# codgodtao/TMDiff

Measured on AMD Instinct MI355X. Metric: UNet denoise-steps/sec (8-ch 64x64, batch 32), higher is better.
Workload: dtype f32; 1 GPU; BASELINE configs[1]: batch-32 8-ch 64x64 tiles, DDPM p_sample steps of the T=1000 cosine schedule, channel_multiplier [32,64,128,256], full UNet forward (both branches) + fused DDPM update per step; batch_per_gpu=32, parallelism=batch-parallel x1, weights=key-hashed random init, text_embedding=fixed synthetic 768-d

## Files before the change

include/tmdiff_hip.h:

```cpp
#ifndef TMDIFF_HIP_H
#define TMDIFF_HIP_H

#include <stddef.h>
#include <stdint.h>

#ifdef __cplusplus
extern "C" {
#endif

#define TMDIFF_ABI_VERSION 6

#define TMDIFF_OK 0
#define TMDIFF_E_INVALID (-1)
#define TMDIFF_E_UNSUPPORTED (-2)
#define TMDIFF_E_LAUNCH (-3)

typedef void* tmdiff_stream_t;

int tmdiff_version(void);
const char* tmdiff_last_error_string(void);

typedef struct tmdiff_conv3d_desc {
  int32_t B, N, H, W;
  int32_t Cin, Cout;
// ... 81 lines not shown
int tmdiff_conv3d_wino_fwd(const tmdiff_conv3d_desc* d, void* workspace, tmdiff_stream_t stream);
int tmdiff_conv3d_wino_fwd_stage(const tmdiff_conv3d_desc* d, void* workspace, int32_t stage, tmdiff_stream_t stream);
int tmdiff_conv3d_wino_fwd_xp(const tmdiff_conv3d_desc* d, void* workspace, int32_t stage, float* xp_out, tmdiff_stream_t stream);
int tmdiff_conv3d_wino_fwd_planes(const tmdiff_conv3d_desc* d, void* workspace, int32_t stage, float* xp_out, int32_t planes,
                                  tmdiff_stream_t stream);

int tmdiff_conv3d_wf_supported(const tmdiff_conv3d_desc* d);
int64_t tmdiff_conv3d_wf_blocks(const tmdiff_conv3d_desc* d);
size_t tmdiff_conv3d_wf_splitk_workspace_bytes(const tmdiff_conv3d_desc* d);
size_t tmdiff_conv3d_wf_workspace_bytes(const tmdiff_conv3d_desc* d);
int32_t tmdiff_conv3d_wf_plan(int32_t B, int32_t Cin, int32_t Cout, int32_t N, int32_t H, int32_t W, int32_t groups, int32_t llm,
                              int64_t* tiles);
int tmdiff_conv3d_wf_fwd(const tmdiff_conv3d_desc* d, void* workspace, tmdiff_stream_t stream);

int tmdiff_conv3d_w2_supported(const tmdiff_conv3d_desc* d);
size_t tmdiff_conv3d_w2_workspace_bytes(const tmdiff_conv3d_desc* d);
size_t tmdiff_conv3d_w2_packed_bytes(int32_t Cout, int32_t Cin);
int tmdiff_conv3d_w2_pack_weights(const float* w, float* packed, int32_t Cout, int32_t Cin, tmdiff_stream_t stream);
int tmdiff_conv3d_w2_fwd(const tmdiff_conv3d_desc* d, void* workspace, int32_t stages, tmdiff_stream_t stream);
int tmdiff_conv3d_wfll_supported(const tmdiff_conv3d_desc* d);
size_t tmdiff_conv3d_wfll_packed_bytes(int32_t Cout, int32_t Cin);
int tmdiff_conv3d_wfll_pack_weights(const float* w, float* packed, int32_t Cout, int32_t Cin, float ll_scale,
                                    tmdiff_stream_t stream);
size_t tmdiff_conv3d_wfll_splitk_workspace_bytes(const tmdiff_conv3d_desc* d);
int tmdiff_conv3d_wfll_fwd(const tmdiff_conv3d_desc* d, float ll_scale, tmdiff_stream_t stream);

size_t tmdiff_conv3d_packed_bf16_bytes(int32_t Cout, int32_t Cin, int32_t ksize, int32_t groups);
int tmdiff_conv3d_pack_weights_bf16(const float* w, void* packed, int32_t Cout, int32_t Cin, int32_t ksize,
                                    int32_t groups, tmdiff_stream_t stream);
int tmdiff_conv3d_pack_weights_bf16_dgrad(const float* w, void* packed, int32_t Cout, int32_t Cin, int32_t ksize,
// ... 298 lines not shown
```

tmdiff_amd/Hyper_unet_general.py:

```python
import math

import torch
import torch.nn as nn

from . import ops, routing

PROMPTS = ("QB", "WV3", "GF2", "WV2", "WV4")

def synthetic_text_embeddings(seed=1234):
    out = {}
    for k, name in enumerate(PROMPTS):
        g = torch.Generator(device="cpu").manual_seed(seed + k)
        out[name] = torch.randn(1, 768, generator=g)
    return out


class Swish(nn.Module):

    def forward(self, x):
        raise RuntimeError("Swish is fused into the HIP kernels; it is never called as a module")



_MASK_FN = None
# ... 402 lines not shown
            y, y2 = self._conv(P, name + ".conv21", [t1], use_bias=False, residual=res, emit=emit, **self._own(pro21), **rckw)
            return (y, y2, None, plan.s2d) if want_ll else (y, y2)
        if side is not None:
            t1p = self._conv(P, name + ".conv20", [side], keep_y=False, emit=pro21)
        elif pre is not None:
            t1p = self._conv(P, name + ".conv20", [pre], keep_y=False, emit=pro21, x_bf16_shape=shape if pre.dtype == torch.int16 else None)
        else:
            t1p = self._conv(P, name + ".conv20", segs, keep_y=False, emit=pro21, **self._own(pro20))
        if plan.emit_ll:
            y2, yll = self._conv(P, name + ".conv21", [t1p], use_bias=False, residual=res, keep_y=False, emit=dict(emit, ll=True), **rckw)
            return None, y2, yll, plan.s2d
        y, y2 = self._conv(P, name + ".conv21", [t1p], use_bias=False, residual=res, emit=emit,
                           x_bf16_shape=shape if name + ".conv21" in P["bf16"] else None, **rckw)
        return (y, y2, None, plan.s2d) if want_ll else (y, y2)

    def _conv0(self, P, name, x, pre):
        if pre is None:
            return self._conv(P, name + ".Conv_0", [x], in_act=True, w2=False)
        return self._conv(P, name + ".Conv_0", [pre], x_bf16_shape=tuple(x.shape[2:]) if pre.dtype == torch.int16 else None, w2=False)

    def _down(self, P, S, name, x, flag, want_high, pre=None, emit=None, fuse=False, xq=None, s2d=False):
        shape = x.shape if x is not None else (*xq.shape[:3], 2 * xq.shape[3], 2 * xq.shape[4])
        plan = self._down_plan(P, name, shape, not want_high, pre is not None and pre.dtype == torch.float32, s2d, fuse)
        pro = self._spec(P, S, shift=None if flag else name + ".Dense_0", scale=name + ".dense1")
        if plan.conv0 == "dwt":
            hll, *bands = self._conv(P, name + ".Conv_0", [pre], keep_y=False, emit=dict(pro, dwt=True))
        elif plan.conv0 is None:
            hh = self._conv0(P, name, x, pre)
        rc2 = {}
        if not ops.config.conv2_after_ll:
            xll = ops.haar_dwt2d(self._conv(P, name + ".Conv_2", [x]), want_high=False, ll_scale=0.5)[0]
        else:
            if xq is None:
                xq = ops.haar_dwt2d(x, want_high=False, ll_scale=0.5)[0]
            if plan.fold:
                c2 = self.get_submodule(name + ".Conv_2")
                xll, rc2 = None, {"res_conv": (xq, c2.weight.detach(), xq.shape[1]), "bias": c2.bias.detach()}
            else:
                xll = self._conv(P, name + ".Conv_2", [xq])
        p16 = False
        if plan.conv0 in ("ll", "wfll"):
            c0, wfll = self.get_submodule(name + ".Conv_0"), plan.conv0 == "wfll"
            hll = (ops.conv3d_wf_ll if wfll else ops.conv3d_ll)(pre, P["w_wfll" if wfll else "w_ll"][name + ".Conv_0"], c0.out_channels, 0.5,
# ... 233 lines not shown
```

tmdiff_amd/_lib.py:

```python
import ctypes as C
import os

_HERE = os.path.dirname(os.path.abspath(__file__))
LIB_PATH = os.environ.get("TMDIFF_HIP_LIB") or os.path.join(_HERE, "libtmdiff_hip.so")

c_float_p = C.POINTER(C.c_float)
vp = C.c_void_p


class Conv3dDesc(C.Structure):
    _fields_ = [
        ("B", C.c_int32), ("N", C.c_int32), ("H", C.c_int32), ("W", C.c_int32),
        ("Cin", C.c_int32), ("Cout", C.c_int32),
        ("groups", C.c_int32), ("ksize", C.c_int32), ("nseg", C.c_int32),
        ("seg_c", C.c_int32 * 3),
        ("seg_x", vp * 3),
        ("w_packed", vp), ("bias", vp), ("bias_scale", C.c_float),
        ("in_shift", vp), ("in_scale", vp), ("in_shift_stride", C.c_int32), ("in_scale_stride", C.c_int32),
        ("in_mask", vp), ("in_act", C.c_int32),
        ("residual", vp), ("out_scale", C.c_float),
        ("y", vp),
        ("y2", vp), ("y2_shift", vp), ("y2_scale", vp), ("y2_shift_stride", C.c_int32), ("y2_scale_stride", C.c_int32),
        ("y2_act", C.c_int32), ("y2_bf16", C.c_int32), ("x_bf16", C.c_int32),
        ("splitk_ws", vp), ("splitk_ws_bytes", C.c_int64),
# ... 16 lines not shown
    "tmdiff_conv3d_fwd_staged": (C.c_int, [C.POINTER(Conv3dDesc), vp, vp]),
    "tmdiff_conv3d_wino_supported": (C.c_int, [C.POINTER(Conv3dDesc)]),
    "tmdiff_conv3d_wino_blocks": (C.c_int64, [C.POINTER(Conv3dDesc)]),
    "tmdiff_conv3d_wino_workspace_bytes": (C.c_size_t, [C.POINTER(Conv3dDesc)]),
    "tmdiff_conv3d_wino_planes": (C.c_int32, [C.c_int32]),
    "tmdiff_conv3d_wino_packed_bytes": (C.c_size_t, [C.c_int32, C.c_int32, C.c_int32, C.c_int32]),
    "tmdiff_conv3d_wino_pack_weights": (C.c_int, [vp, vp, C.c_int32, C.c_int32, C.c_int32, C.c_int32, C.c_int32, vp]),
    "tmdiff_conv3d_wino_pack_weights_multi_chunk": (C.c_int32, []),
    "tmdiff_conv3d_wino_pack_weights_multi": (C.c_int, [vp, vp, vp, C.c_int32, vp]),
    "tmdiff_conv3d_wf_supported": (C.c_int, [C.POINTER(Conv3dDesc)]),
    "tmdiff_conv3d_wf_blocks": (C.c_int64, [C.POINTER(Conv3dDesc)]),
    "tmdiff_conv3d_wf_workspace_bytes": (C.c_size_t, [C.POINTER(Conv3dDesc)]),
    "tmdiff_conv3d_wf_splitk_workspace_bytes": (C.c_size_t, [C.POINTER(Conv3dDesc)]),
    "tmdiff_conv3d_wf_fwd": (C.c_int, [C.POINTER(Conv3dDesc), vp, vp]),
    "tmdiff_conv3d_w2_supported": (C.c_int, [C.POINTER(Conv3dDesc)]),
    "tmdiff_conv3d_w2_workspace_bytes": (C.c_size_t, [C.POINTER(Conv3dDesc)]),
    "tmdiff_conv3d_w2_packed_bytes": (C.c_size_t, [C.c_int32, C.c_int32]),
    "tmdiff_conv3d_w2_pack_weights": (C.c_int, [vp, vp, C.c_int32, C.c_int32, vp]),
    "tmdiff_conv3d_w2_fwd": (C.c_int, [C.POINTER(Conv3dDesc), vp, C.c_int32, vp]),
    "tmdiff_conv3d_wino_fwd": (C.c_int, [C.POINTER(Conv3dDesc), vp, vp]),
    "tmdiff_conv3d_wino_fwd_planes": (C.c_int, [C.POINTER(Conv3dDesc), vp, C.c_int32, vp, C.c_int32, vp]),
    "tmdiff_conv3d_wino_fwd_xp": (C.c_int, [C.POINTER(Conv3dDesc), vp, C.c_int32, vp, vp]),
    "tmdiff_conv3d_wino_fwd_stage": (C.c_int, [C.POINTER(Conv3dDesc), vp, C.c_int32, vp]),
    "tmdiff_conv3d_prologue_fwd": (C.c_int, [C.POINTER(Conv3dDesc), vp, vp]),
    "tmdiff_conv3d_ll_supported": (C.c_int, [C.POINTER(Conv3dDesc)]),
    "tmdiff_conv3d_ll_splitk_workspace_bytes": (C.c_size_t, [C.POINTER(Conv3dDesc)]),
    "tmdiff_conv3d_ll_packed_bytes": (C.c_size_t, [C.c_int32, C.c_int32]),
    "tmdiff_conv3d_ll_pack_weights": (C.c_int, [vp, vp, C.c_int32, C.c_int32, C.c_float, vp]),
    "tmdiff_conv3d_ll_fwd": (C.c_int, [C.POINTER(Conv3dDesc), C.c_float, vp]),
    "tmdiff_conv3d_packed_bf16_bytes": (C.c_size_t, [C.c_int32, C.c_int32, C.c_int32, C.c_int32]),
# ... 189 lines not shown
```

tmdiff_amd/csrc/conv3d_w2.hip:

```cpp
#include "bufaddr.h"
#include "common.h"

namespace {

using namespace tmdiff;

constexpr int W2_XP = 384;
constexpr int W2_NP = 256;
constexpr int W2_KC = 16;
constexpr int W2_CO = 64;

struct W2Plan {
  int T, Q, TW, Hp, IP, OP;
  int G, ptiles;
  size_t xh_floats, mh_floats;
};

bool w2_shape_ok(const tmdiff_conv3d_desc* d) {
  if (!d || d->ksize != 3 || d->groups != 1 || d->x_bf16 || d->y2_bf16 || d->nseg != 1) return false;
  if (d->B <= 0 || (d->N != 4 && d->N != 8) || d->W < 2 || d->W > 16 || d->W % 2 || d->H < 4 || d->H > 32) return false;
  if (d->Cin < 128 || d->Cin % 32 || d->Cout < 256 || d->Cout % W2_CO || d->seg_c[0] != d->Cin) return false;
  if (d->in_mask || d->drop_p > 0.f || d->rc_x || d->rc_cin || d->y_ll || d->y_hi[0] || d->y2_s2d || d->xp_out) return false;
  return true;
}

W2Plan w2_plan(const tmdiff_conv3d_desc* d) {
  W2Plan p;
  p.T = d->N / 4; p.Q = d->B * p.T; p.TW = d->W / 2; p.Hp = d->H + 2;
  p.IP = p.Hp * p.TW; p.OP = d->H * p.TW;
  p.G = W2_NP / p.OP < W2_XP / p.IP ? W2_NP / p.OP : W2_XP / p.IP;
  if (p.G > p.Q) p.G = p.Q;
  p.ptiles = (p.Q + p.G - 1) / p.G;
  p.xh_floats = (size_t)24 * d->Cin * p.Q * p.IP;
  p.mh_floats = (size_t)24 * d->Cout * p.Q * p.OP;
  return p;
}

bool w2_fits(const tmdiff_conv3d_desc* d, const W2Plan& p) {
  const size_t xk = p.xh_floats / 24 * 4, mk = p.mh_floats / 24 * 4, uk = (size_t)3 * d->Cin * d->Cout * 4;
  return xk < (1ull << 31) && mk < (1ull << 31) && uk < (1ull << 31) && p.Q <= 65535 &&
         (long)p.ptiles * (d->Cout / W2_CO) * 24 < 0x7fffffffL;
}

__global__ void __launch_bounds__(256) w2_pack_kernel(const float* __restrict__ w, float* __restrict__ u, int Cout, int Cin) {
#pragma clang fp contract(off)
  const long idx = (long)blockIdx.x * 256 + threadIdx.x;
  if (idx >= (long)3 * Cin * Cout) return;
  const int e = idx & 3;
  long r = idx >> 2;
  const int co = r % Cout; r /= Cout;
  const int cq = r % (Cin / 4);
  const int dh = r / (Cin / 4);
  const int ci = cq * 4 + e;
  const float* src = w + ((long)co * Cin + ci) * 27 + dh * 3;
  float t[6][3];
// ... 211 lines not shown
}

struct W2OutArgs {
  const float* mh;
  const float* bias;
  float bias_scale;
  const float* residual;
  float out_scale;
  float* y;
  float* y2;
  const float* y2_shift;
  const float* y2_scale;
  int y2_shift_stride, y2_scale_stride, y2_act;
  int Cout, N, H, W, T, TW, OP;
  long QOP;
};

template <bool Y, bool RES, bool Y2>
__global__ void __launch_bounds__(256) w2_output_kernel(const W2OutArgs a) {
#pragma clang fp contract(off)
  __shared__ float tile[4 * 32 * 17];
  const int tid = threadIdx.x;
  const int cc = blockIdx.x, h = blockIdx.y, q = blockIdx.z;
  const int b = q / a.T, t = q % a.T;
  {
    const int co_l = tid & 31, tw = tid >> 5;
    if (tw < a.TW) {
      const float* src = a.mh + ((long)q * a.OP + h * a.TW + tw) * a.Cout + cc * 32 + co_l;
      const long kstride = a.QOP * a.Cout;
      float r[6][2];
// ... 39 lines not shown
    if constexpr (Y2) {
      const float sh2 = a.y2_shift ? a.y2_shift[(long)b * a.y2_shift_stride + co] : 0.f;
      const float sc2 = a.y2_scale ? a.y2_scale[(long)b * a.y2_scale_stride + co] : 1.f;
      float u[2];
#pragma unroll
      for (int e = 0; e < 2; ++e) {
        const float x = v[e] + sh2;
        const float xa = silu_f(x);
        u[e] = (a.y2_act ? xa : x) * sc2;
      }
      buf::store2(r2, o, make_float2(u[0], u[1]));
    }
  }
}

}

extern "C" int tmdiff_conv3d_w2_supported(const tmdiff_conv3d_desc* d) {
  return w2_shape_ok(d) && w2_fits(d, w2_plan(d)) ? 1 : 0;
}

extern "C" size_t tmdiff_conv3d_w2_workspace_bytes(const tmdiff_conv3d_desc* d) {
  if (!w2_shape_ok(d)) return 0;
  const W2Plan p = w2_plan(d);
  return (p.xh_floats + p.mh_floats) * sizeof(float);
}

extern "C" size_t tmdiff_conv3d_w2_packed_bytes(int32_t Cout, int32_t Cin) {
  if (Cout <= 0 || Cin <= 0 || Cin % 4) return 0;
  return (size_t)72 * Cout * Cin * sizeof(float);
}

extern "C" int tmdiff_conv3d_w2_pack_weights(const float* w, float* packed, int32_t Cout, int32_t Cin, tmdiff_stream_t stream) {
  using namespace tmdiff;
  TMDIFF_REQUIRE(w && packed, "conv3d_w2_pack_weights: NULL pointer");
  TMDIFF_REQUIRE(Cout > 0 && Cin > 0 && Cin % 4 == 0 && (size_t)72 * Cout * Cin < (1ull << 31),
                 "conv3d_w2_pack_weights: Cout=%d Cin=%d (Cin %% 4 == 0)", Cout, Cin);
  const long n = (long)3 * Cin * Cout;
  w2_pack_kernel<<<(unsigned)((n + 255) / 256), 256, 0, as_stream(stream)>>>(w, packed, Cout, Cin);
  return check_launch("conv3d_w2_pack_weights");
}

extern "C" int tmdiff_conv3d_w2_fwd(const tmdiff_conv3d_desc* d, void* workspace, int32_t stages, tmdiff_stream_t stream) {
  using namespace tmdiff;
  TMDIFF_REQUIRE(d && workspace, "conv3d_w2_fwd: NULL pointer");
  if (!w2_shape_ok(d))
    return fail(TMDIFF_E_UNSUPPORTED, "conv3d_w2_fwd: fp32 3x3x3, groups 1, one input tensor, 4 or 8 bands, even W <= 16, 4 <= H <= 32, "
                                      "Cin >= 128 (%% 32), Cout >= 256 (%% 64), plain y / y2 / residual epilogue");
  const W2Plan p = w2_plan(d);
  if (!w2_fits(d, p)) return fail(TMDIFF_E_UNSUPPORTED, "conv3d_w2_fwd: tensor too large for 32-bit offsets");
  TMDIFF_REQUIRE(d->seg_x[0] && d->w_packed && (d->y || d->y2), "conv3d_w2_fwd: input, weights and an output");
  TMDIFF_REQUIRE(aligned16(d->seg_x[0]) && aligned16(workspace) && aligned16(d->w_packed) && aligned16(d->y) && aligned16(d->y2) &&
                     aligned16(d->residual),
                 "conv3d_w2_fwd: 16-byte aligned tensors / workspace");
  hipStream_t st = as_stream(stream);
  float* xh = static_cast<float*>(workspace);
  float* mh = xh + p.xh_floats;
  if (stages == 0) stages = 7;

  if (stages & 1) {
    W2InArgs a;
    a.x = d->seg_x[0]; a.xh = xh;
    a.in_shift = d->in_shift; a.in_scale = d->in_scale;
    a.shift_stride = bank_stride(d->in_shift_stride, d->Cin);
    a.scale_stride = bank_stride(d->in_scale_stride, d->Cin);
    a.in_act = d->in_act;
    a.Cin = d->Cin; a.N = d->N; a.H = d->H; a.W = d->W; a.T = p.T; a.TW = p.TW; a.IP = p.IP;
    a.QIP = (long)p.Q * p.IP;
    w2_input_kernel<<<dim3((unsigned)(d->Cin / 32), (unsigned)p.Hp, (unsigned)p.Q), 256, 0, st>>>(a);
// ... 5 lines not shown
    a.Cin = d->Cin; a.Cout = d->Cout; a.Q = p.Q; a.TW = p.TW; a.IP = p.IP; a.OP = p.OP; a.G = p.G; a.ptiles = p.ptiles;
    a.cotiles = d->Cout / W2_CO;
    if (const int rc = set_grid(a, (long)p.ptiles * a.cotiles * 24, "conv3d_w2_fwd")) return rc;
    w2_gemm_kernel<<<a.total_blocks, 256, 0, st>>>(a);
    if (const int rc = check_launch("conv3d_w2_fwd")) return rc;
  }
  if (stages & 4) {
    W2OutArgs a;
    a.mh = mh;
    a.bias = d->bias; a.bias_scale = d->bias_scale; a.residual = d->residual; a.out_scale = d->out_scale;
    a.y = d->y; a.y2 = d->y2; a.y2_shift = d->y2_shift; a.y2_scale = d->y2_scale; a.y2_act = d->y2_act;
    a.y2_shift_stride = bank_stride(d->y2_shift_stride, d->Cout);
    a.y2_scale_stride = bank_stride(d->y2_scale_stride, d->Cout);
    a.Cout = d->Cout; a.N = d->N; a.H = d->H; a.W = d->W; a.T = p.T; a.TW = p.TW; a.OP = p.OP;
    a.QOP = (long)p.Q * p.OP;
    const dim3 grid((unsigned)(d->Cout / 32), (unsigned)d->H, (unsigned)p.Q);
#define TMDIFF_W2_OUT(Y, R, Y2) w2_output_kernel<Y, R, Y2><<<grid, 256, 0, st>>>(a)
    if (d->y) {
      if (d->residual) { if (d->y2) TMDIFF_W2_OUT(true, true, true); else TMDIFF_W2_OUT(true, true, false); }
      else             { if (d->y2) TMDIFF_W2_OUT(true, false, true); else TMDIFF_W2_OUT(true, false, false); }
    } else {
      if (d->residual) TMDIFF_W2_OUT(false, true, true); else TMDIFF_W2_OUT(false, false, true);
    }
#undef TMDIFF_W2_OUT
    if (const int rc = check_launch("conv3d_w2_fwd(output pass)")) return rc;
  }
  return TMDIFF_OK;
}
```

tmdiff_amd/ops.py:

```python
import collections
import ctypes as C
import math
import os

import numpy as np
import torch

from . import _lib, routing
from ._lib import Conv3dDesc, check, lib



class KernelConfig:

    _FLAG = lambda default: (lambda v: (v != "0") if default else (v == "1"))
    _FIELDS = {
        "winograd": ("TMDIFF_WINOGRAD", _FLAG(True), True), "wf": ("TMDIFF_WF", _FLAG(True), True),
        "wf_pair": ("TMDIFF_WF_PAIR", _FLAG(True), True), "wf_splitk": ("TMDIFF_WF_SPLITK", _FLAG(True), True),
        "wf_min_fill": ("TMDIFF_WF_MIN_FILL", float, 0.7), "wino_min_blocks": ("TMDIFF_WINO_MIN_BLOCKS", int, 256),
        "ll_compose": ("TMDIFF_LL_COMPOSE", _FLAG(True), True), "wfll": ("TMDIFF_WFLL", _FLAG(True), True),
        "train_ll_wino": ("TMDIFF_TRAIN_LL_WINO", _FLAG(True), True),
        "conv2_after_ll": ("TMDIFF_CONV2_AFTER_LL", _FLAG(True), True),
        "epilogue_fuse": ("TMDIFF_EPILOGUE_FUSE", _FLAG(True), True), "producer_fuse": ("TMDIFF_PRODUCER_FUSE", _FLAG(True), True),
        "fp32_staged": ("TMDIFF_FP32_STAGED", str, "auto"), "bf16_pack": ("TMDIFF_BF16_PACK", str, "auto"),
        "wgrad_wino": ("TMDIFF_WGRAD_WINO", _FLAG(True), True), "wgrad_wino_bias": ("TMDIFF_WGRAD_WINO_BIAS", _FLAG(True), True),
        "wgrad_bias": ("TMDIFF_WGRAD_BIAS", _FLAG(False), False), "wino_multipack": ("TMDIFF_WINO_MULTIPACK", _FLAG(True), True),
        "fuse_res_conv": ("TMDIFF_FUSE_RES_CONV", _FLAG(True), True), "emit_ll": ("TMDIFF_EMIT_LL", _FLAG(True), True),
        "emit_dwt": ("TMDIFF_EMIT_DWT", _FLAG(True), True), "side_xp": ("TMDIFF_SIDE_XP", _FLAG(True), True),
        "train_fused_resblock": ("TMDIFF_TRAIN_FUSED_RESBLOCK", _FLAG(True), True),
        "train_graph": ("TMDIFF_TRAIN_GRAPH", _FLAG(False), False),
        "train_two_streams": ("TMDIFF_TRAIN_STREAMS", _FLAG(True), True),
        "sample_graph": ("TMDIFF_SAMPLE_GRAPH", _FLAG(False), False),
        "grad_bf16": ("TMDIFF_GRAD_BF16", _FLAG(False), False),
        "wino2d": ("TMDIFF_WINO2D", _FLAG(True), True),
    }

    def __init__(self, env=None):
        env = os.environ if env is None else env
        for name, (var, parse, default) in self._FIELDS.items():
            object.__setattr__(self, name, parse(env[var]) if var in env else default)

    def __setattr__(self, name, value):
        if name not in self._FIELDS:
            raise AttributeError(f"ops.config has no switch {name!r}")
        object.__setattr__(self, name, value)

    def key(self):
        return tuple(getattr(self, n) for n in self._FIELDS)

# ... 448 lines not shown
    e1.record()
    rec = (e0, e1, flops, ksize, what, _tag(d) + suffix)
    TIMER.records.append(rec if bytes_of is None else rec + (bytes_of(d),))


def _conv3d_bytes(d):
    y2_b = 0.0 if not d.y2 else (2.0 if d.y2_bf16 else 4.0)
    return d.B * d.N * d.H * d.W * ((2.0 if d.x_bf16 else 4.0) * d.Cin +
                                    d.Cout * (4.0 * ((1 if d.y else 0) + (1 if d.residual else 0)) + y2_b) +
                                    (4.0 * d.Cin if d.xp_out else 0.0))


def conv3d(segs, w_packed, cout, ksize, out=None, math="fp32", pack_input=None, staged=None, emit=None, keep_y=True,
           x_bf16_shape=None, xp_out=None, **kw):
    if kw.get("res_conv") is not None or kw.get("y_ll") is not None or (emit is not None and (emit.get("ll") or emit.get("dwt"))):
        raise ValueError("conv3d: only conv3d_wf folds a residual convolution into its epilogue / writes the LL band")
    b, _, n, h, w = segs[0].shape if x_bf16_shape is None else (segs[0].shape[0], None, *x_bf16_shape)
    dev = segs[0].device
    bf16 = math == "bf16"
    y, y2 = _outputs("conv3d", dev, (b, cout, n, h, w), keep_y, emit,
                     (b, cout // 8, n * h * w, 8) if bf16 else (b, cout, n, h, w), torch.int16 if bf16 else torch.float32, out)
    d = make_conv_desc(segs, w_packed, cout, ksize, y, y2=y2, x_bf16_shape=x_bf16_shape, **kw, **_emit_kw(emit))
    if d.xp_out and (math != "fp32" or not lib.tmdiff_conv3d_fwd_xp_supported(C.byref(d))):
        raise ValueError("conv3d: side_xp needs the 16-byte 1x1x1 bandwidth kernel (ask routing.k1_side_xp first)")
    if bf16:
        if w_packed.dtype != torch.int16:
            raise TypeError("conv3d(math='bf16') needs weights from pack_conv_weight_bf16")
        if pack_input is None:
            pack_input = {"0": False, "1": True}.get(config.bf16_pack, True)
        nb = lib.tmdiff_conv3d_bf16_workspace_bytes(C.byref(d))
        ws = _workspace(dev, nb).data_ptr() if pack_input and ksize == 3 and x_bf16_shape is None and nb else None
# ... 55 lines not shown
    def __init__(self, direct, wf=None, wino=None, w2=None):
        self.direct, self.wf, self.wino, self.w2 = direct, wf, wino, w2


def conv3d_auto(segs, weights, cout, groups=1, math="fp32", emit=None, keep_y=True, xp_out=None, x_bf16_shape=None, family=None,
                **kw):
    if math == "bf16" or x_bf16_shape is not None:
        return conv3d(segs, weights.direct(), cout, 3, groups=groups, math=math, emit=emit, keep_y=keep_y,
                      x_bf16_shape=x_bf16_shape, **kw)
    b, _, n, h, w = segs[0].shape
    cin = sum(s_.shape[1] for s_ in segs)
    masked, dropout, plain = kw.get("in_mask") is not None, kw.get("drop") is not None, _plain(segs, kw)
    fam = family or routing.conv3_family(b, cin, cout, n, h, w, groups, plain=plain, masked=masked, dropout=dropout,
                                         keep_xp=xp_out is not None)
    if (fam in ("wf", "wf_pair") and weights.w2 is not None and family is None and xp_out is None and len(segs) == 1 and
            not masked and not dropout and kw.get("res_conv") is None and
            not (emit is not None and (emit.get("s2d") or emit.get("ll") or emit.get("dwt"))) and
            routing.wino2d_route(b, cin, cout, n, h, w, groups)):
        return conv3d_w2(segs[0], weights.w2(), cout, emit=emit, keep_y=keep_y, **kw)
    if fam in ("wf", "wf_pair") and weights.wf is not None:
        return conv3d_wf(segs, weights.wf(), cout, emit=emit, keep_y=keep_y, groups=groups, xp_out=xp_out, **kw)
    if fam in ("wino4", "wino2") and weights.wino is not None:
        from . import fallback
        planes = 6 if fam == "wino4" else 4
        return fallback.conv3d_wino(segs, weights.wino(planes), cout, planes, emit=emit, keep_y=keep_y, groups=groups,
                                    xp_out=xp_out, **kw)
    if (emit is not None and (emit.get("s2d") or emit.get("ll") or emit.get("dwt"))) or kw.get("res_conv") is not None:
        raise ValueError("conv3d_auto: only conv3d_wf writes a space-to-depth second output / folds a residual convolution "
                         "(ask routing.wf_route first)")
    if fam not in ("staged", "fused"):
        fam = routing.direct_family(cin, cout, groups, plain, masked, dropout, xp_out is not None, extents=(b, n, h, w))
    return conv3d(segs, weights.direct(), cout, 3, groups=groups, staged=fam == "staged", emit=emit, keep_y=keep_y,
                  xp_out=xp_out, **kw)


def conv3d_wf(segs, w_packed, cout, emit=None, keep_y=True, groups=1, xp_out=None, **kw):
    b, _, n, h, w = segs[0].shape
    dev = segs[0].device
    s2d = bool(emit is not None and emit.get("s2d"))
    want_ll = bool(emit is not None and emit.get("ll"))
    want_dwt = bool(emit is not None and emit.get("dwt"))
    if want_dwt and (s2d or want_ll):
        raise ValueError("conv3d_wf: emit dwt=True excludes s2d / ll")
# ... 24 lines not shown


def pack_conv_weight_w2(w):
    cout, cin = w.shape[0], w.shape[1]
    nb = lib.tmdiff_conv3d_w2_packed_bytes(cout, cin)
    if tuple(w.shape[2:]) != (3, 3, 3) or nb == 0:
        raise ValueError(f"pack_conv_weight_w2: weight shape {tuple(w.shape)} not supported")
    out = torch.empty(nb // 4, device=w.device, dtype=torch.float32)
    check(lib.tmdiff_conv3d_w2_pack_weights(_chk(w.detach(), "w"), out.data_ptr(), cout, cin, stream_ptr()), "conv3d_w2_pack_weights")
    return out


def conv3d_w2(x, w_packed, cout, emit=None, keep_y=True, stages=0, **kw):
    b, _, n, h, w = x.shape
    dev = x.device
    if emit is not None and (emit.get("s2d") or emit.get("ll") or emit.get("dwt")):
        raise ValueError("conv3d_w2: no space-to-depth / LL / Haar outputs (conv3d_wf writes those)")
    y, y2 = _outputs("conv3d_w2", dev, (b, cout, n, h, w), keep_y, emit, (b, cout, n, h, w))
    d = make_conv_desc([x], w_packed, cout, 3, y, y2=y2, **kw, **_emit_kw(emit))
    if not lib.tmdiff_conv3d_w2_supported(C.byref(d)):
        raise ValueError("conv3d_w2: shape not supported (routing.wino2d_ok)")
    nws = lib.tmdiff_conv3d_w2_workspace_bytes(C.byref(d))
    ws = _workspace(dev, nws, "w2").data_ptr()
    _launch(lib.tmdiff_conv3d_w2_fwd, d, (ws, int(stages)), "conv3d_w2_fwd", "conv3d_w2_fwd", 2.0 * b * cout * d.Cin * 9.0 * n * h * w)
    return _result(y, y2)


def pack_conv_weight_ll(w, ll_scale=0.5):
    cout, cin = w.shape[0], w.shape[1]
    nb = lib.tmdiff_conv3d_ll_packed_bytes(cout, cin)
    if tuple(w.shape[2:]) != (3, 3, 3) or nb == 0:
        raise ValueError(f"pack_conv_weight_ll: weight shape {tuple(w.shape)} not supported")
    out = torch.empty(nb // 4, device=w.device, dtype=torch.float32)
    check(lib.tmdiff_conv3d_ll_pack_weights(_chk(w.detach(), "w"), out.data_ptr(), cout, cin, float(ll_scale), stream_ptr()),
          "conv3d_ll_pack_weights")
    return out


def conv3d_ll(x, w_packed, cout, ll_scale=0.5, emit=None, keep_y=True, **kw):
    b, _, n, h, w = x.shape
# ... 1454 lines not shown
```

tmdiff_amd/routing.py:

```python
import collections
import ctypes as C

from . import _lib
from ._lib import lib

PRODUCT_FAMILIES = ("wf", "wf_pair", "wfll", "ll", "staged", "fused", "bf16")
FALLBACK_FAMILIES = ("wino4", "wino2")


def _config():
    from . import ops
    return ops.config


def _grad_bf16():
    return bool(getattr(_config(), "grad_bf16", False))


def wino_weight_ok(cout, cin, ksize=3, groups=1):
    return (ksize == 3 and groups in (1, 3) and cin % groups == 0 and cout % groups == 0 and (cin // groups) % 2 == 0 and
            (cout // groups) % 32 == 0)


def staged_weight_ok(cout, cin, groups=1):
# ... 60 lines not shown

def wino2d_ok(b, cin, cout, n, h, w, groups=1):
    if groups != 1 or b <= 0 or n not in (4, 8) or w < 2 or w > 16 or w % 2 or h < 4 or h > 32:
        return False
    if cin < 128 or cin % 32 or cout < 256 or cout % 64:
        return False
    q, tw = b * (n // 4), w // 2
    ip, op = (h + 2) * tw, h * tw
    g = max(1, min(q, 256 // op, 384 // ip))
    return (4 * cin * q * ip < (1 << 31) and 4 * cout * q * op < (1 << 31) and 12 * cin * cout < (1 << 31) and q <= 65535 and
            ((q + g - 1) // g) * (cout // 64) * 24 < 0x7fffffff)


def wino2d_route(b, cin, cout, n, h, w, groups=1):
    return bool(_config().wino2d and wino2d_ok(b, cin, cout, n, h, w, groups))


def wfll_route(b, cin, cout, n, h, w):
    if not (_config().wfll and n in (4, 8) and h % 2 == 0 and w % 8 == 0 and cout % 32 == 0):
        return False
    return wf_route(b, 4 * cin, cout, n, h // 2, w // 2, llm=True)[0]


def wino_plan(b, cout, n, h, w, groups=1, cin=None):
    planes = lib.tmdiff_conv3d_wino_planes(int(n))
    if not planes or w % 4:
        return 0, 0
    if cin is not None and not supported("tmdiff_conv3d_wino_supported", b, cin, cout, n, h, w, groups):
        return 0, 0
    cg = cout // groups
# ... 411 lines not shown
```

Measured before the change: 45.93 batch32-steps/s.

## Extend Winograd-2D conv epilogue to fold 1x1x1 residual conv and LL/Haar/s2d outputs

Adds a second output-transform kernel to the Winograd 2D (w2) conv path. It can fold a 1x1x1 residual convolution computed with MFMA, and it can write LL, Haar-band and space-to-depth quarter-resolution outputs. Routing now sends these epilogue-bearing convs and the down-block Conv_0 to w2 instead of the wf kernel. The aim is to use the faster w2 path for more layers and avoid separate kernels or tensors for the DWT and residual conv. In exchange the output kernel is more complex, and it uses half-height tiles with an extra MFMA loop.

```diff
diff --git a/include/tmdiff_hip.h b/include/tmdiff_hip.h
--- a/include/tmdiff_hip.h
+++ b/include/tmdiff_hip.h
@@ -119,6 +119,7 @@
 int tmdiff_conv3d_wf_fwd(const tmdiff_conv3d_desc* d, void* workspace, tmdiff_stream_t stream);
 
 int tmdiff_conv3d_w2_supported(const tmdiff_conv3d_desc* d);
+int tmdiff_conv3d_w2_epilogue_supported(const tmdiff_conv3d_desc* d);
 size_t tmdiff_conv3d_w2_workspace_bytes(const tmdiff_conv3d_desc* d);
 size_t tmdiff_conv3d_w2_packed_bytes(int32_t Cout, int32_t Cin);
 int tmdiff_conv3d_w2_pack_weights(const float* w, float* packed, int32_t Cout, int32_t Cin, tmdiff_stream_t stream);
diff --git a/tmdiff_amd/Hyper_unet_general.py b/tmdiff_amd/Hyper_unet_general.py
--- a/tmdiff_amd/Hyper_unet_general.py
+++ b/tmdiff_amd/Hyper_unet_general.py
@@ -440,10 +440,10 @@
                            x_bf16_shape=shape if name + ".conv21" in P["bf16"] else None, **rckw)
         return (y, y2, None, plan.s2d) if want_ll else (y, y2)
 
-    def _conv0(self, P, name, x, pre):
+    def _conv0(self, P, name, x, pre, w2=False):
         if pre is None:
-            return self._conv(P, name + ".Conv_0", [x], in_act=True, w2=False)
-        return self._conv(P, name + ".Conv_0", [pre], x_bf16_shape=tuple(x.shape[2:]) if pre.dtype == torch.int16 else None, w2=False)
+            return self._conv(P, name + ".Conv_0", [x], in_act=True, w2=w2)
+        return self._conv(P, name + ".Conv_0", [pre], x_bf16_shape=tuple(x.shape[2:]) if pre.dtype == torch.int16 else None, w2=w2)
 
     def _down(self, P, S, name, x, flag, want_high, pre=None, emit=None, fuse=False, xq=None, s2d=False):
         shape = x.shape if x is not None else (*xq.shape[:3], 2 * xq.shape[3], 2 * xq.shape[4])
@@ -452,7 +452,9 @@
         if plan.conv0 == "dwt":
             hll, *bands = self._conv(P, name + ".Conv_0", [pre], keep_y=False, emit=dict(pro, dwt=True))
         elif plan.conv0 is None:
-            hh = self._conv0(P, name, x, pre)
+            c0 = self.get_submodule(name + ".Conv_0")
+            hh = self._conv0(P, name, x, pre, w2=want_high and not ops.config.emit_dwt and routing.wino2d_epilogue_route(
+                shape[0], c0.in_channels, c0.out_channels, *shape[2:], quarter=True))
         rc2 = {}
         if not ops.config.conv2_after_ll:
             xll = ops.haar_dwt2d(self._conv(P, name + ".Conv_2", [x]), want_high=False, ll_scale=0.5)[0]
diff --git a/tmdiff_amd/_lib.py b/tmdiff_amd/_lib.py
--- a/tmdiff_amd/_lib.py
+++ b/tmdiff_amd/_lib.py
@@ -54,6 +54,7 @@
     "tmdiff_conv3d_wf_splitk_workspace_bytes": (C.c_size_t, [C.POINTER(Conv3dDesc)]),
     "tmdiff_conv3d_wf_fwd": (C.c_int, [C.POINTER(Conv3dDesc), vp, vp]),
     "tmdiff_conv3d_w2_supported": (C.c_int, [C.POINTER(Conv3dDesc)]),
+    "tmdiff_conv3d_w2_epilogue_supported": (C.c_int, [C.POINTER(Conv3dDesc)]),
     "tmdiff_conv3d_w2_workspace_bytes": (C.c_size_t, [C.POINTER(Conv3dDesc)]),
     "tmdiff_conv3d_w2_packed_bytes": (C.c_size_t, [C.c_int32, C.c_int32]),
     "tmdiff_conv3d_w2_pack_weights": (C.c_int, [vp, vp, C.c_int32, C.c_int32, vp]),
diff --git a/tmdiff_amd/csrc/conv3d_w2.hip b/tmdiff_amd/csrc/conv3d_w2.hip
--- a/tmdiff_amd/csrc/conv3d_w2.hip
+++ b/tmdiff_amd/csrc/conv3d_w2.hip
@@ -16,11 +16,35 @@
   size_t xh_floats, mh_floats;
 };
 
-bool w2_shape_ok(const tmdiff_conv3d_desc* d) {
+bool w2_extents_ok(const tmdiff_conv3d_desc* d) {
   if (!d || d->ksize != 3 || d->groups != 1 || d->x_bf16 || d->y2_bf16 || d->nseg != 1) return false;
   if (d->B <= 0 || (d->N != 4 && d->N != 8) || d->W < 2 || d->W > 16 || d->W % 2 || d->H < 4 || d->H > 32) return false;
   if (d->Cin < 128 || d->Cin % 32 || d->Cout < 256 || d->Cout % W2_CO || d->seg_c[0] != d->Cin) return false;
-  if (d->in_mask || d->drop_p > 0.f || d->rc_x || d->rc_cin || d->y_ll || d->y_hi[0] || d->y2_s2d || d->xp_out) return false;
+  if (d->in_mask || d->drop_p > 0.f || d->xp_out) return false;
+  return true;
+}
+
+bool w2_folds(const tmdiff_conv3d_desc* d) { return d->rc_x || d->rc_w || d->rc_cin; }
+bool w2_quarter(const tmdiff_conv3d_desc* d) { return d->y_ll || d->y_hi[0] || d->y_hi[1] || d->y_hi[2] || d->y2_s2d; }
+
+bool w2_shape_ok(const tmdiff_conv3d_desc* d) { return w2_extents_ok(d) && !w2_folds(d) && !w2_quarter(d); }
+
+bool w2_epilogue_ok(const tmdiff_conv3d_desc* d) {
+  if (!w2_extents_ok(d)) return false;
+  if (!w2_folds(d) && !w2_quarter(d)) return true;
+  if (d->H % 2) return false;
+  if (w2_quarter(d) && d->N != 8) return false;
+  if (d->y_ll) {
+    const bool dwt = d->y_hi[0] != nullptr;
+    if (d->y || (dwt ? (d->y2 || d->y2_s2d || !d->y_hi[1] || !d->y_hi[2]) : !d->y2)) return false;
+  } else if (d->y_hi[0] || d->y_hi[1] || d->y_hi[2]) {
+    return false;
+  }
+  if (d->y2_s2d && !d->y2) return false;
+  if (w2_folds(d)) {
+    if (!d->rc_x || d->rc_cin <= 0 || d->rc_cin % 32 || d->rc_cin > 512 || d->residual) return false;
+    if ((long)d->rc_cin * d->N * d->H * d->W >= (1L << 30)) return false;
+  }
   return true;
 }
 
@@ -38,7 +62,8 @@
 
 bool w2_fits(const tmdiff_conv3d_desc* d, const W2Plan& p) {
   const size_t xk = p.xh_floats / 24 * 4, mk = p.mh_floats / 24 * 4, uk = (size_t)3 * d->Cin * d->Cout * 4;
-  return xk < (1ull << 31) && mk < (1ull << 31) && uk < (1ull << 31) && p.Q <= 65535 &&
+  const size_t yk = (size_t)32 * d->N * d->H * d->W * 4;
+  return xk < (1ull << 31) && mk < (1ull << 31) && uk < (1ull << 31) && yk < (1ull << 31) && p.Q <= 65535 &&
          (long)p.ptiles * (d->Cout / W2_CO) * 24 < 0x7fffffffL;
 }
 
@@ -280,6 +305,12 @@
   int y2_shift_stride, y2_scale_stride, y2_act;
   int Cout, N, H, W, T, TW, OP;
   long QOP;
+  float* y_ll;
+  float* y_hi[3];
+  int y2_s2d;
+  const float* rc_x;
+  const float* rc_w;
+  int rc_cin;
 };
 
 template <bool Y, bool RES, bool Y2>
@@ -349,14 +380,178 @@
   }
 }
 
+constexpr int W2_RS = 32 * 17 + 16;
+
+template <bool RES, bool RC>
+__global__ void __launch_bounds__(256) w2_output2_kernel(const W2OutArgs a) {
+#pragma clang fp contract(off)
+  __shared__ float tile[8 * W2_RS];
+  const int tid = threadIdx.x;
+  const int lane = tid & 63, wv = __builtin_amdgcn_readfirstlane(tid >> 6);
+  const int l31 = lane & 31, khalf = lane >> 5;
+  const int cc = blockIdx.x, hp = blockIdx.y, q = blockIdx.z;
+  const int b = q / a.T, t = q % a.T;
+  const int hw = a.H * a.W;
+  const long plane = (long)a.N * hw;
+
+  const int ngrp = RC ? a.rc_cin / 32 : 0;
+  const buf::rsrc xr = buf::make(RC ? a.rc_x + (long)b * a.rc_cin * plane : nullptr, RC ? (unsigned)((long)a.rc_cin * plane * 4) : 0u);
+  const int rrow = l31 >> 4, rcol = l31 & 15;
+  const unsigned xo = (unsigned)((4 * khalf * (int)plane + (rcol < a.W ? ((4 * t + wv) * a.H + 2 * hp + rrow) * a.W + rcol : 0)) * 4);
+  const unsigned ch_bytes = (unsigned)(plane * 4);
+  const float* wrow = RC ? a.rc_w + (long)(cc * 32 + l31) * a.rc_cin + 4 * khalf : nullptr;
+  float4 aw0[4], aw1[4];
+  float xv0[16], xv1[16];
+  auto fetch = [&](int jg, float4 (&aw)[4], float (&xv)[16]) __attribute__((always_inline)) {
+#pragma unroll
+    for (int i = 0; i < 4; ++i) aw[i] = *reinterpret_cast<const float4*>(wrow + jg * 32 + 8 * i);
+#pragma unroll
+    for (int i = 0; i < 4; ++i)
+#pragma unroll
+      for (int e = 0; e < 4; ++e) xv[4 * i + e] = buf::load(xr, xo, (unsigned)(jg * 32 + 8 * i + e) * ch_bytes);
+  };
+  if constexpr (RC) fetch(0, aw0, xv0);
+
+  {
+    const int co_l = tid & 31, tw = tid >> 5;
+    if (tw < a.TW) {
+      const long kstride = a.QOP * a.Cout;
+#pragma unroll
+      for (int row = 0; row < 2; ++row) {
+        const float* src = a.mh + ((long)q * a.OP + (2 * hp + row) * a.TW + tw) * a.Cout + cc * 32 + co_l;
+        float r[6][2];
+#pragma unroll
+        for (int kb = 0; kb < 6; ++kb) {
+          const float m0 = src[(kb * 4 + 0) * kstride], m1 = src[(kb * 4 + 1) * kstride], m2 = src[(kb * 4 + 2) * kstride],
+                      m3 = src[(kb * 4 + 3) * kstride];
+          r[kb][0] = (m0 + m1) + m2;
+          r[kb][1] = (m1 - m2) - m3;
+        }
+#pragma unroll
+        for (int j = 0; j < 2; ++j) {
+          const float p12 = r[1][j] + r[2][j], d12 = r[1][j] - r[2][j], p34 = r[3][j] + r[4][j], d34 = r[3][j] - r[4][j];
+          float* dst = tile + row * W2_RS + co_l * 17 + 2 * tw + j;
+          dst[0 * 2 * W2_RS] = (r[0][j] + p12) + p34;
+          dst[1 * 2 * W2_RS] = d12 + 2.f * d34;
+          dst[2 * 2 * W2_RS] = p12 + 4.f * p34;
+          dst[3 * 2 * W2_RS] = (d12 + 8.f * d34) + r[5][j];
+        }
+      }
+    }
+  }
+  __syncthreads();
+
+  if constexpr (RC) {
+    float* const tb = tile + (wv * 2 + rrow) * W2_RS + 4 * khalf * 17 + rcol;
+    f32x16 acc;
+#pragma unroll
+    for (int r = 0; r < 16; ++r) acc[r] = tb[((r & 3) + 8 * (r >> 2)) * 17];
+    auto mma = [&](const float4 (&aw)[4], const float (&xv)[16]) __attribute__((always_inline)) {
+#pragma unroll
+      for (int i = 0; i < 4; ++i) {
+        acc = __builtin_amdgcn_mfma_f32_32x32x2f32(aw[i].x, xv[4 * i + 0], acc, 0, 0, 0);
+        acc = __builtin_amdgcn_mfma_f32_32x32x2f32(aw[i].y, xv[4 * i + 1], acc, 0, 0, 0);
+        acc = __builtin_amdgcn_mfma_f32_32x32x2f32(aw[i].z, xv[4 * i + 2], acc, 0, 0, 0);
+        acc = __builtin_amdgcn_mfma_f32_32x32x2f32(aw[i].w, xv[4 * i + 3], acc, 0, 0, 0);
+      }
+    };
+    for (int jg = 0; jg < ngrp; jg += 2) {
+      if (jg + 1 < ngrp) fetch(jg + 1, aw1, xv1);
+      mma(aw0, xv0);
+      if (jg + 1 < ngrp) {
+        if (jg + 2 < ngrp) fetch(jg + 2, aw0, xv0);
+        mma(aw1, xv1);
+      }
+    }
+#pragma unroll
+    for (int r = 0; r < 16; ++r) tb[((r & 3) + 8 * (r >> 2)) * 17] = acc[r];
+    __syncthreads();
+  }
+
+  const long cb = ((long)b * a.Cout + cc * 32) * plane;
+  const unsigned span = (unsigned)(32 * plane * 4);
+  const bool want_y = a.y != nullptr, want_y2 = a.y2 != nullptr, want_ll = a.y_ll != nullptr, want_hi = a.y_hi[0] != nullptr;
+  const buf::rsrc ry = buf::make(want_y ? a.y + cb : nullptr, want_y ? span : 0u);
+  const buf::rsrc rr = buf::make(RES ? a.residual + cb : nullptr, RES ? span : 0u);
+  const buf::rsrc r2 = buf::make(want_y2 ? a.y2 + cb : nullptr, want_y2 ? span : 0u);
+  const long cbq = cb >> 2;
+  const unsigned spanq = span >> 2;
+  const buf::rsrc rll = buf::make(want_ll ? a.y_ll + cbq : nullptr, want_ll ? spanq : 0u);
+  const buf::rsrc rh0 = buf::make(want_hi ? a.y_hi[0] + cbq : nullptr, want_hi ? spanq : 0u);
+  const buf::rsrc rh1 = buf::make(want_hi ? a.y_hi[1] + cbq : nullptr, want_hi ? spanq : 0u);
+  const buf::rsrc rh2 = buf::make(want_hi ? a.y_hi[2] + cbq : nullptr, want_hi ? spanq : 0u);
+  const int hq = a.H >> 1, wq = a.W >> 1;
+#pragma unroll
+  for (int it = 0; it < 4; ++it) {
+    const int i = tid + 256 * it;
+    const int wp = i & 7, band = (i >> 3) & 3, co_l = i >> 5;
+    const int co = cc * 32 + co_l;
+    const int n = 4 * t + band;
+    const bool ok = wp < a.TW;
+    const unsigned o0 = ok ? (unsigned)(((co_l * a.N + n) * a.H + 2 * hp) * a.W + 2 * wp) * 4u : buf::kOutside;
+    const unsigned o1 = buf::at(o0, (unsigned)a.W * 4u);
+    const unsigned oq = ok ? (unsigned)(((co_l * a.N + n) * hq + hp) * wq + wp) * 4u : buf::kOutside;
+    const float* s = tile + band * 2 * W2_RS + co_l * 17 + 2 * wp;
+    float v[4] = {s[0], s[1], s[W2_RS], s[W2_RS + 1]};
+    const float bias_t = a.bias ? a.bias[co] * a.bias_scale : 0.f;
+    float2 res0 = make_float2(0.f, 0.f), res1 = make_float2(0.f, 0.f);
+    if constexpr (RES) res0 = buf::load2(rr, o0), res1 = buf::load2(rr, o1);
+    v[0] = (v[0] + bias_t + res0.x) * a.out_scale;
+    v[1] = (v[1] + bias_t + res0.y) * a.out_scale;
+    v[2] = (v[2] + bias_t + res1.x) * a.out_scale;
+    v[3] = (v[3] + bias_t + res1.y) * a.out_scale;
+    if (want_y) {
+      buf::store2(ry, o0, make_float2(v[0], v[1]));
+      buf::store2(ry, o1, make_float2(v[2], v[3]));
+    }
+    const float sh2 = a.y2_shift ? a.y2_shift[(long)b * a.y2_shift_stride + co] : 0.f;
+    const float sc2 = a.y2_scale ? a.y2_scale[(long)b * a.y2_scale_stride + co] : 1.f;
+    if (want_y2) {
+      float u[4];
+#pragma unroll
+      for (int e = 0; e < 4; ++e) {
+        const float x = v[e] + sh2;
+        const float xa = silu_f(x);
+        u[e] = (a.y2_act ? xa : x) * sc2;
+      }
+      if (a.y2_s2d) {
+        const unsigned os = ok ? (unsigned)(((4 * co_l * a.N + n) * hq + hp) * wq + wp) * 4u : buf::kOutside;
+        const unsigned qplane4 = (unsigned)(plane >> 2) * 4u;
+#pragma unroll
+        for (int e = 0; e < 4; ++e) buf::store(r2, buf::at(os, (unsigned)e * qplane4), u[e]);
+      } else {
+        buf::store2(r2, o0, make_float2(u[0], u[1]));
+        buf::store2(r2, o1, make_float2(u[2], u[3]));
+      }
+    }
+    if (want_ll) {
+      const float ll = ((v[0] + v[1]) + (v[2] + v[3])) * 0.25f;
+      if (want_hi) {
+        const float x = ll + sh2;
+        const float xa = silu_f(x);
+        buf::store(rll, oq, (a.y2_act ? xa : x) * sc2);
+        buf::store(rh0, oq, ((v[0] - v[1]) + (v[2] - v[3])) * 0.5f);
+        buf::store(rh1, oq, ((v[0] + v[1]) - (v[2] + v[3])) * 0.5f);
+        buf::store(rh2, oq, ((v[0] - v[1]) - (v[2] - v[3])) * 0.5f);
+      } else {
+        buf::store(rll, oq, ll);
+      }
+    }
+  }
+}
+
 }
 
 extern "C" int tmdiff_conv3d_w2_supported(const tmdiff_conv3d_desc* d) {
   return w2_shape_ok(d) && w2_fits(d, w2_plan(d)) ? 1 : 0;
 }
 
+extern "C" int tmdiff_conv3d_w2_epilogue_supported(const tmdiff_conv3d_desc* d) {
+  return w2_epilogue_ok(d) && w2_fits(d, w2_plan(d)) ? 1 : 0;
+}
+
 extern "C" size_t tmdiff_conv3d_w2_workspace_bytes(const tmdiff_conv3d_desc* d) {
-  if (!w2_shape_ok(d)) return 0;
+  if (!w2_epilogue_ok(d)) return 0;
   const W2Plan p = w2_plan(d);
   return (p.xh_floats + p.mh_floats) * sizeof(float);
 }
@@ -379,15 +574,18 @@
 extern "C" int tmdiff_conv3d_w2_fwd(const tmdiff_conv3d_desc* d, void* workspace, int32_t stages, tmdiff_stream_t stream) {
   using namespace tmdiff;
   TMDIFF_REQUIRE(d && workspace, "conv3d_w2_fwd: NULL pointer");
-  if (!w2_shape_ok(d))
+  if (!w2_epilogue_ok(d))
     return fail(TMDIFF_E_UNSUPPORTED, "conv3d_w2_fwd: fp32 3x3x3, groups 1, one input tensor, 4 or 8 bands, even W <= 16, 4 <= H <= 32, "
-                                      "Cin >= 128 (%% 32), Cout >= 256 (%% 64), plain y / y2 / residual epilogue");
+                                      "Cin >= 128 (%% 32), Cout >= 256 (%% 64); a folded 1x1x1 (rc_cin %% 32 == 0, at most 512, no residual) "
+                                      "and LL / Haar / space-to-depth outputs (8 bands) on even H");
   const W2Plan p = w2_plan(d);
   if (!w2_fits(d, p)) return fail(TMDIFF_E_UNSUPPORTED, "conv3d_w2_fwd: tensor too large for 32-bit offsets");
-  TMDIFF_REQUIRE(d->seg_x[0] && d->w_packed && (d->y || d->y2), "conv3d_w2_fwd: input, weights and an output");
+  TMDIFF_REQUIRE(d->seg_x[0] && d->w_packed && (d->y || d->y2 || d->y_ll), "conv3d_w2_fwd: input, weights and an output");
   TMDIFF_REQUIRE(aligned16(d->seg_x[0]) && aligned16(workspace) && aligned16(d->w_packed) && aligned16(d->y) && aligned16(d->y2) &&
-                     aligned16(d->residual),
+                     aligned16(d->residual) && aligned16(d->y_ll) && aligned16(d->y_hi[0]) && aligned16(d->y_hi[1]) &&
+                     aligned16(d->y_hi[2]) && aligned16(d->rc_x) && aligned16(d->rc_w),
                  "conv3d_w2_fwd: 16-byte aligned tensors / workspace");
+  TMDIFF_REQUIRE(!d->rc_x || d->rc_w, "conv3d_w2_fwd: rc_x without rc_w");
   hipStream_t st = as_stream(stream);
   float* xh = static_cast<float*>(workspace);
   float* mh = xh + p.xh_floats;
@@ -423,9 +621,17 @@
     a.y2_scale_stride = bank_stride(d->y2_scale_stride, d->Cout);
     a.Cout = d->Cout; a.N = d->N; a.H = d->H; a.W = d->W; a.T = p.T; a.TW = p.TW; a.OP = p.OP;
     a.QOP = (long)p.Q * p.OP;
+    a.y_ll = d->y_ll; a.y2_s2d = d->y2 && d->y2_s2d ? 1 : 0;
+    for (int i = 0; i < 3; ++i) a.y_hi[i] = d->y_hi[0] ? d->y_hi[i] : nullptr;
+    a.rc_x = d->rc_x; a.rc_w = d->rc_w; a.rc_cin = d->rc_cin;
     const dim3 grid((unsigned)(d->Cout / 32), (unsigned)d->H, (unsigned)p.Q);
 #define TMDIFF_W2_OUT(Y, R, Y2) w2_output_kernel<Y, R, Y2><<<grid, 256, 0, st>>>(a)
-    if (d->y) {
+    if (w2_folds(d) || w2_quarter(d)) {
+      const dim3 grid2((unsigned)(d->Cout / 32), (unsigned)(d->H / 2), (unsigned)p.Q);
+      if (d->rc_x) w2_output2_kernel<false, true><<<grid2, 256, 0, st>>>(a);
+      else if (d->residual) w2_output2_kernel<true, false><<<grid2, 256, 0, st>>>(a);
+      else w2_output2_kernel<false, false><<<grid2, 256, 0, st>>>(a);
+    } else if (d->y) {
       if (d->residual) { if (d->y2) TMDIFF_W2_OUT(true, true, true); else TMDIFF_W2_OUT(true, true, false); }
       else             { if (d->y2) TMDIFF_W2_OUT(true, false, true); else TMDIFF_W2_OUT(true, false, false); }
     } else {
diff --git a/tmdiff_amd/ops.py b/tmdiff_amd/ops.py
--- a/tmdiff_amd/ops.py
+++ b/tmdiff_amd/ops.py
@@ -33,6 +33,7 @@
         "sample_graph": ("TMDIFF_SAMPLE_GRAPH", _FLAG(False), False),
         "grad_bf16": ("TMDIFF_GRAD_BF16", _FLAG(False), False),
         "wino2d": ("TMDIFF_WINO2D", _FLAG(True), True),
+        "wino2d_epilogue": ("TMDIFF_WINO2D_EPILOGUE", _FLAG(True), True),
     }
 
     def __init__(self, env=None):
@@ -511,7 +512,7 @@
 def conv3d(segs, w_packed, cout, ksize, out=None, math="fp32", pack_input=None, staged=None, emit=None, keep_y=True,
            x_bf16_shape=None, xp_out=None, **kw):
     if kw.get("res_conv") is not None or kw.get("y_ll") is not None or (emit is not None and (emit.get("ll") or emit.get("dwt"))):
-        raise ValueError("conv3d: only conv3d_wf folds a residual convolution into its epilogue / writes the LL band")
+        raise ValueError("conv3d: only conv3d_wf / conv3d_w2 fold a residual convolution into their epilogue / write the LL band")
     b, _, n, h, w = segs[0].shape if x_bf16_shape is None else (segs[0].shape[0], None, *x_bf16_shape)
     dev = segs[0].device
     bf16 = math == "bf16"
@@ -597,10 +598,12 @@
     fam = family or routing.conv3_family(b, cin, cout, n, h, w, groups, plain=plain, masked=masked, dropout=dropout,
                                          keep_xp=xp_out is not None)
     if (fam in ("wf", "wf_pair") and weights.w2 is not None and family is None and xp_out is None and len(segs) == 1 and
-            not masked and not dropout and kw.get("res_conv") is None and
-            not (emit is not None and (emit.get("s2d") or emit.get("ll") or emit.get("dwt"))) and
-            routing.wino2d_route(b, cin, cout, n, h, w, groups)):
-        return conv3d_w2(segs[0], weights.w2(), cout, emit=emit, keep_y=keep_y, **kw)
+            not masked and not dropout):
+        rc = kw.get("res_conv")
+        quarter = bool(emit is not None and (emit.get("s2d") or emit.get("ll") or emit.get("dwt")))
+        if (routing.wino2d_epilogue_route(b, cin, cout, n, h, w, groups, int(rc[2]) if rc is not None else 0, quarter)
+                if (rc is not None or quarter) else routing.wino2d_route(b, cin, cout, n, h, w, groups)):
+            return conv3d_w2(segs[0], weights.w2(), cout, emit=emit, keep_y=keep_y, **kw)
     if fam in ("wf", "wf_pair") and weights.wf is not None:
         return conv3d_wf(segs, weights.wf(), cout, emit=emit, keep_y=keep_y, groups=groups, xp_out=xp_out, **kw)
     if fam in ("wino4", "wino2") and weights.wino is not None:
@@ -609,7 +612,7 @@
         return fallback.conv3d_wino(segs, weights.wino(planes), cout, planes, emit=emit, keep_y=keep_y, groups=groups,
                                     xp_out=xp_out, **kw)
     if (emit is not None and (emit.get("s2d") or emit.get("ll") or emit.get("dwt"))) or kw.get("res_conv") is not None:
-        raise ValueError("conv3d_auto: only conv3d_wf writes a space-to-depth second output / folds a residual convolution "
+        raise ValueError("conv3d_auto: only conv3d_wf / conv3d_w2 write a space-to-depth second output / fold a residual convolution "
                          "(ask routing.wf_route first)")
     if fam not in ("staged", "fused"):
         fam = routing.direct_family(cin, cout, groups, plain, masked, dropout, xp_out is not None, extents=(b, n, h, w))
@@ -664,16 +667,35 @@
 def conv3d_w2(x, w_packed, cout, emit=None, keep_y=True, stages=0, **kw):
     b, _, n, h, w = x.shape
     dev = x.device
-    if emit is not None and (emit.get("s2d") or emit.get("ll") or emit.get("dwt")):
-        raise ValueError("conv3d_w2: no space-to-depth / LL / Haar outputs (conv3d_wf writes those)")
-    y, y2 = _outputs("conv3d_w2", dev, (b, cout, n, h, w), keep_y, emit, (b, cout, n, h, w))
-    d = make_conv_desc([x], w_packed, cout, 3, y, y2=y2, **kw, **_emit_kw(emit))
-    if not lib.tmdiff_conv3d_w2_supported(C.byref(d)):
-        raise ValueError("conv3d_w2: shape not supported (routing.wino2d_ok)")
+    s2d = bool(emit is not None and emit.get("s2d"))
+    want_ll = bool(emit is not None and emit.get("ll"))
+    want_dwt = bool(emit is not None and emit.get("dwt"))
+    if want_dwt and (s2d or want_ll):
+        raise ValueError("conv3d_w2: emit dwt=True excludes s2d / ll")
+    want_ll = want_ll or want_dwt
+    if want_ll and keep_y:
+        raise ValueError("conv3d_w2: the LL output replaces y (keep_y=False)")
+    rc = kw.get("res_conv")
+    if rc is not None and kw.get("residual") is not None:
+        raise ValueError("conv3d_w2: res_conv excludes a residual tensor")
+    if (s2d or want_ll or rc is not None) and not routing.wino2d_epilogue_ok(b, x.shape[1], cout, n, h, w, 1,
+                                                                             int(rc[2]) if rc is not None else 0, s2d or want_ll):
+        raise ValueError("conv3d_w2: this launch cannot fold a 1x1x1 / write a space-to-depth / LL output "
+                         "(ask routing.wino2d_epilogue_ok first)")
+    q = (b, cout, n, h // 2, w // 2)
+    y_ll = torch.empty(*q, device=dev, dtype=torch.float32) if want_ll else None
+    y_hi = [torch.empty(*q, device=dev, dtype=torch.float32) for _ in range(3)] if want_dwt else None
+    y, y2 = _outputs("conv3d_w2", dev, (b, cout, n, h, w), keep_y, emit,
+                     None if want_dwt else ((b, 4 * cout, n, h // 2, w // 2) if s2d else (b, cout, n, h, w)))
+    d = make_conv_desc([x], w_packed, cout, 3, y, y2=y2, y2_s2d=s2d, y_ll=y_ll, y_hi=y_hi, **kw, **_emit_kw(emit))
+    if not lib.tmdiff_conv3d_w2_epilogue_supported(C.byref(d)):
+        raise ValueError("conv3d_w2: shape not supported (routing.wino2d_ok / wino2d_epilogue_ok)")
     nws = lib.tmdiff_conv3d_w2_workspace_bytes(C.byref(d))
     ws = _workspace(dev, nws, "w2").data_ptr()
-    _launch(lib.tmdiff_conv3d_w2_fwd, d, (ws, int(stages)), "conv3d_w2_fwd", "conv3d_w2_fwd", 2.0 * b * cout * d.Cin * 9.0 * n * h * w)
-    return _result(y, y2)
+    flops = 2.0 * b * cout * (d.Cin * 9.0 + d.rc_cin) * n * h * w
+    _launch(lib.tmdiff_conv3d_w2_fwd, d, (ws, int(stages)), "conv3d_w2_fwd", "conv3d_w2_fwd", flops, 3,
+            f" +rc{d.rc_cin}" if d.rc_cin else "")
+    return (y_ll, *y_hi) if want_dwt else (y2, y_ll) if want_ll else _result(y, y2)
 
 
 def pack_conv_weight_ll(w, ll_scale=0.5):
diff --git a/tmdiff_amd/routing.py b/tmdiff_amd/routing.py
--- a/tmdiff_amd/routing.py
+++ b/tmdiff_amd/routing.py
@@ -98,6 +98,21 @@
 
 def wino2d_route(b, cin, cout, n, h, w, groups=1):
     return bool(_config().wino2d and wino2d_ok(b, cin, cout, n, h, w, groups))
+
+
+def wino2d_epilogue_ok(b, cin, cout, n, h, w, groups=1, rc_cin=0, quarter=False):
+    if not wino2d_ok(b, cin, cout, n, h, w, groups):
+        return False
+    if not rc_cin and not quarter:
+        return True
+    if h % 2 or (quarter and n != 8):
+        return False
+    return not rc_cin or (rc_cin > 0 and rc_cin % 32 == 0 and rc_cin <= 512 and rc_cin * n * h * w < (1 << 30))
+
+
+def wino2d_epilogue_route(b, cin, cout, n, h, w, groups=1, rc_cin=0, quarter=False):
+    cfg = _config()
+    return bool(cfg.wino2d and cfg.wino2d_epilogue and wino2d_epilogue_ok(b, cin, cout, n, h, w, groups, rc_cin, quarter))
 
 
 def wfll_route(b, cin, cout, n, h, w):
```

After: 46.99 batch32-steps/s, median of 6. 2.3% higher.
